# JuliaReinforcementLearning/ReinforcementLearning.jl

Hardware: NVIDIA H100
Metric: env-steps/sec at 65536 CartPole envs (full PPO iteration: rollout T=32 + GAE + 4 epochs x 4 minibatches) (higher is better)
Workload: dtype f32

## Files before the change

reinforcementlearning.jl_b200/csrc/nn_tc.cu:

```cuda
#include "nn.cuh"
#include "perm.cuh"
#include "tc_split.h"
#include "wgmma.cuh"

namespace {

constexpr int NT = 256;
constexpr int TM = 128;
constexpr int H = 64;
constexpr int G_F = 128;
constexpr int GW_S = 8 * G_F;
constexpr int WIMG_BYTES = 16 * GW_S;
constexpr float kScaleW = 64.0f;
constexpr float kLog2Pi = 1.8378770664093453f;

__device__ __forceinline__ float act_f(int act, float z) { return act == B200RL_ACT_RELU ? fmaxf(z, 0.f) : tanhf(z); }
__device__ __forceinline__ void split2(float a, float b, uint32_t& hi, uint32_t& lo) {
    const __half2 h = __floats2half2_rn(a, b);
    const float2 back = __half22float2(h);
    const __half2 l = __floats2half2_rn(a - back.x, b - back.y);
    hi = *reinterpret_cast<const uint32_t*>(&h);
    lo = *reinterpret_cast<const uint32_t*>(&l);
}
__device__ __forceinline__ float half_bits_to_float(uint32_t bits16) { return __half2float(__ushort_as_half((unsigned short)bits16)); }
__device__ __forceinline__ float softplus_f(float x) { return x > 0.f ? x + log1pf(expf(-x)) : log1pf(expf(x)); }
__device__ __forceinline__ float normlogpdf1(float mu, float sigma, float x) {
    float s = sigma + 1e-8f, v = s * s, dd = x - mu;
    return -0.5f * ((logf(v) + (dd * dd) / v) + kLog2Pi);
}
__device__ __forceinline__ uint32_t wimg_off(int n, int k) { return (uint32_t)((n >> 3) * GW_S + (k >> 3) * G_F + (n & 7) * 16 + (k & 7) * 2); }

constexpr int NT7 = 512;
constexpr int GF_T = 128;
constexpr int GS_T = 16 * GF_T;
constexpr int FIMG = 8 * GS_T;
constexpr float kScaleH = 64.0f, kScaleX = 64.0f;
constexpr int kNo = 2;

struct SmemBwd {
    static_assert(FIMG % 128 == 0 && WIMG_BYTES % 128 == 0 && (2 * GS_T) % 16 == 0, "operand images must stay 128-byte aligned");
    alignas(128) uint8_t FP_full[FIMG];
    alignas(128) uint8_t FP_lo[FIMG];
    alignas(128) uint8_t FH_lo[FIMG];
    alignas(128) uint8_t FH_full[FIMG];
    alignas(16) uint8_t FH_ones[2 * GS_T];
    alignas(128) uint8_t FQ_full[FIMG];
    alignas(128) uint8_t FQ_lo[FIMG];
    alignas(128) uint8_t B1[WIMG_BYTES];
    alignas(128) uint8_t XT[2][2 * GS_T];
    alignas(128) uint8_t AH_full[FIMG];
    alignas(128) uint8_t AH_lo[FIMG];
    alignas(16) float D[TM * H];
    float W1[kInMax * H];
    float b1[H], b2[H];
    float W3[H * kNo];
    float b3[kNo];
    float Zp[4 * kNo * TM];
    float Red[32];
    double RedD[16];
    float step_scale;
    alignas(8) uint64_t bar1;
    alignas(8) uint64_t bar2;
    alignas(8) uint64_t bar3;
    alignas(8) uint64_t bar4;
    float AccW2[64 * 65 + 64];
    float AccD4[64 * 9];
};
__device__ __forceinline__ int d_off(int s, int col) { return s * H + ((((col >> 2) ^ (s & 15))) << 2) + (col & 3); }
__device__ __forceinline__ void d_ld16(const float* D, int s, int f0, float (&v)[16]) {
#pragma unroll
    for (int u = 0; u < 4; ++u) {
        const float4 q4 = *reinterpret_cast<const float4*>(D + d_off(s, f0 + 4 * u));
        v[4 * u] = q4.x; v[4 * u + 1] = q4.y; v[4 * u + 2] = q4.z; v[4 * u + 3] = q4.w;
    }
}
template <int TB>
__device__ __forceinline__ void gemm_ts3(float (&d)[32], const uint8_t* a_hi, const uint8_t* a_lo, int h, uint64_t dB, uint32_t b_step) {
    const uint64_t dA = wg::make_desc(wg::smem_u32(a_hi) + 8 * h * GF_T, GS_T, GF_T), dAl = wg::make_desc(wg::smem_u32(a_lo) + 8 * h * GF_T, GS_T, GF_T);
    wg::fence();
#pragma unroll
    for (int k = 0; k < 4; ++k) {
        const uint32_t aa = k * 2 * GS_T, bb = k * b_step;
        wg::mma_m64n64k16<0, TB>(d, wg::desc_add(dA, aa), wg::desc_add(dB, bb), k ? 1u : 0u);
        wg::mma_m64n64k16<0, TB>(d, wg::desc_add(dA, aa), wg::desc_add(dB, 8 * GW_S + bb), 1u);
        wg::mma_m64n64k16<0, TB>(d, wg::desc_add(dAl, aa), wg::desc_add(dB, bb), 1u);
    }
    wg::commit();
    wg::wait_all();
}
__device__ __forceinline__ uint32_t fimg_off(int f, int s) { return (uint32_t)((f >> 3) * GS_T + (s >> 3) * GF_T + (s & 7) * 16 + (f & 7) * 2); }
__device__ __forceinline__ void store16_feat(uint8_t* img, int f0, int s, const uint32_t (&v)[8]) {
    uint8_t* p = img + fimg_off(f0, s);
    *reinterpret_cast<uint4*>(p) = make_uint4(v[0], v[1], v[2], v[3]);
    *reinterpret_cast<uint4*>(p + GS_T) = make_uint4(v[4], v[5], v[6], v[7]);
}
__device__ __forceinline__ float dact_f(int act, float h) { return act == B200RL_ACT_RELU ? (h > 0.f ? 1.f : 0.f) : 1.f - h * h; }

__device__ __forceinline__ uint32_t mix32(uint32_t h) {
    h ^= h >> 16; h *= 0x85EBCA6Bu; h ^= h >> 13; h *= 0xC2B2AE35u; h ^= h >> 16;
    return h;
}
using b200perm::perm_index;
using b200perm::perm_index_bits;
__device__ __forceinline__ float block_sum512(float v, float* red) {
#pragma unroll
    for (int o = 16; o > 0; o >>= 1) v += __shfl_xor_sync(0xffffffffu, v, o);
    __syncthreads();
    if ((threadIdx.x & 31) == 0) red[threadIdx.x >> 5] = v;
    __syncthreads();
    float t = 0.f;
    if (threadIdx.x == 0)
        for (int k = 0; k < NT7 / 32; ++k) t += red[k];
    return t;
}
__device__ __forceinline__ float sigmoid_f(float x) { return 1.f / (1.f + expf(-x)); }

__device__ __forceinline__ float lane_transpose_reduce32(float (&v)[32], int lane) {
#pragma unroll
    for (int st = 0; st < 5; ++st) {
        const int half = 16 >> st, off = 16 >> st;
        const bool upper = (lane & off) != 0;
#pragma unroll
        for (int n = 0; n < half; ++n) {
            float send = upper ? v[n] : v[n + half];
            float keep = upper ? v[n + half] : v[n];
            v[n] = keep + __shfl_xor_sync(0xffffffffu, send, off);
        }
    }
    return v[0];
}

__device__ __forceinline__ void worker_sync() { asm volatile("bar.sync 1, 512;" ::: "memory"); }
__device__ __forceinline__ void group_sync(int q) { asm volatile("bar.sync %0, 128;" ::"r"(5 + q) : "memory"); }
__device__ __forceinline__ void ready_arrive(int id) { asm volatile("bar.arrive %0, 640;" ::"r"(id) : "memory"); }
__device__ __forceinline__ void ready_wait(int id) { asm volatile("bar.sync %0, 640;" ::"r"(id) : "memory"); }
struct LossOut { float dz[kNo]; float l0, l1; };
__device__ __forceinline__ LossOut sample_loss(const MlpDesc& actor, int role, const AcHyper& hp, float inv_B, const float (&z)[kNo],
                                               float a_bits, float lp_old, float A, float ret) {
    LossOut r;
#pragma unroll
    for (int o = 0; o < kNo; ++o) r.dz[o] = 0.f;
    r.l0 = 0.f; r.l1 = 0.f;
    if (role == 1) {
        float err = ret - z[0];
        r.l0 = err * err;
        r.dz[0] = -2.0f * hp.w_critic * inv_B * err;
        return r;
    }
    float logp_a, gsel;
    if (!actor.heads2) {
        int na = actor.nout;
        float lp[kNo], pr[kNo];
        float m = -3.4e38f;
#pragma unroll
        for (int o = 0; o < kNo; ++o) if (o < na) m = fmaxf(m, z[o]);
        float se = 0.f;
#pragma unroll
        for (int o = 0; o < kNo; ++o) if (o < na) se += expf(z[o] - m);
        float ls = logf(se);
        float Hent = 0.f;
#pragma unroll
        for (int o = 0; o < kNo; ++o) {
            lp[o] = (z[o] - m) - ls;
            pr[o] = o < na ? expf(lp[o]) : 0.f;
            if (o < na) Hent -= pr[o] * lp[o];
        }
        int a = __float_as_int(a_bits) - 1;
        logp_a = 0.f;
#pragma unroll
        for (int o = 0; o < kNo; ++o) if (o == a) logp_a = lp[o];
        r.l1 = Hent;
        if (hp.algo == 0) {
            float ratio = expf(logp_a - lp_old);
            float u = ratio * A;
            float rc = fminf(fmaxf(ratio, 1.0f - hp.clip_range), 1.0f + hp.clip_range);
            float cc = rc * A;
            r.l0 = -fminf(u, cc);
            bool inside = ratio >= 1.0f - hp.clip_range && ratio <= 1.0f + hp.clip_range;
            gsel = (u < cc || inside) ? u : 0.f;
        } else {
            r.l0 = -(logp_a * A);
            gsel = A;
        }
        float dlogp = -hp.w_actor * inv_B * gsel;
#pragma unroll
        for (int o = 0; o < kNo; ++o)
            if (o < na) r.dz[o] = dlogp * ((o == a ? 1.f : 0.f) - pr[o]) + hp.w_entropy * inv_B * pr[o] * (lp[o] + Hent);
    } else {
        float mu = z[0], raw = z[1];
        float sp = softplus_f(raw);
        float sigma = fminf(fmaxf(sp, hp.min_sigma), hp.max_sigma);
        bool clamped = sp < hp.min_sigma || sp > hp.max_sigma;
        float a = a_bits;
        logp_a = normlogpdf1(mu, sigma, a);
        float Hent = logf(sigma) + 0.5f * (kLog2Pi + 1.0f);
        r.l1 = Hent;
        if (hp.algo == 0) {
            float ratio = expf(logp_a - lp_old);
            float u = ratio * A;
            float rc = fminf(fmaxf(ratio, 1.0f - hp.clip_range), 1.0f + hp.clip_range);
            float cc = rc * A;
            r.l0 = -fminf(u, cc);
            bool inside = ratio >= 1.0f - hp.clip_range && ratio <= 1.0f + hp.clip_range;
            gsel = (u < cc || inside) ? u : 0.f;
        } else {
            r.l0 = -(logp_a * A);
            gsel = A;
        }
        float dlogp = -hp.w_actor * inv_B * gsel;
        float sgm = sigma + 1e-8f, dd = a - mu;
        r.dz[0] = dlogp * (dd / (sgm * sgm));
        float dsig = dlogp * (-1.0f / sgm + (dd * dd) / (sgm * sgm * sgm)) - hp.w_entropy * inv_B * (1.0f / sigma);
        r.dz[1] = clamped ? 0.f : dsig * sigmoid_f(raw);
    }
    return r;
}

#ifdef B200RL_K7_TIMING
__device__ unsigned long long g_k7_phase[40];
__device__ int g_k7_watch = 0;
#define K7_T(i) do { if (tid == (g_k7_watch & 0xFFFF) && (int)blockIdx.x == (g_k7_watch >> 16)) { long long now_ = clock64(); g_k7_phase[i] += (unsigned long long)(now_ - tprev_); tprev_ = now_; } } while (0)
#else
#define K7_T(i) do { } while (0)
#endif
constexpr int NT7_ALL = NT7 + 128;
constexpr int kRegsMma = 64, kRegsWorker = 104;
static_assert(128 * kRegsMma + NT7 * kRegsWorker <= NT7_ALL * 96, "setmaxnreg split must fit the CTA's register allocation");
constexpr int kBarRdyA = 2, kBarRdyB = 3, kBarRdyC = 4;

template <int ACT>
__global__ void __launch_bounds__(NT7_ALL, 1)
ac_loss_grad_tc_kernel(MlpDesc actor, MlpDesc critic, const float* params , AcHyper hp, AcBatch b, float* partial,
                       float* __restrict__ loss_partial, int64_t np_total, float scale_base ,
                       AcStep st ,
                       int n_actor ) {
    extern __shared__ __align__(1024) unsigned char smem_raw[];
    SmemBwd& sm = *reinterpret_cast<SmemBwd*>(smem_raw);
    const int role = (int)blockIdx.x < n_actor ? 0 : 1;
    const int cta = role ? (int)blockIdx.x - n_actor : (int)blockIdx.x;
    const int nctas = role ? (int)gridDim.x - n_actor : n_actor;
    const int nrows = max(n_actor, (int)gridDim.x - n_actor);
    const float scale_p = scale_base * (role ? 4.0f : 64.0f);
    const MlpDesc d = role ? critic : actor;
    const int act = ACT >= 0 ? ACT : d.act;
    const bool relu = act == B200RL_ACT_RELU;
    const int64_t poff = role ? actor.nparams() : 0;
    const float* __restrict__ p = params + poff;
    const int tid = threadIdx.x, warp = tid >> 5, lane = tid & 31;
    const int q = warp & 3, c = (warp >> 2) & 3;
    const int s = 32 * q + lane;
    {
        const float* b1 = p + (int64_t)H * d.in;
        const float* W2 = b1 + H;
        const float* b2 = W2 + (int64_t)H * H;
        const float s1 = relu ? kScaleH : 1.0f;
        for (int k = tid; k < kInMax * H; k += NT7_ALL) sm.W1[k] = (k / H) < d.in ? p[k] * s1 : 0.f;
        for (int k = tid; k < H; k += NT7_ALL) { sm.b1[k] = b1[k] * s1; sm.b2[k] = b2[k]; }
        for (int k = tid; k < H * kNo; k += NT7_ALL) {
            int j = k / kNo, o = k % kNo;
            sm.W3[k] = o < d.nout ? p[head_w<false>(d, o, j)] : 0.f;
        }
        if (tid < kNo) sm.b3[tid] = tid < d.nout ? p[head_b<false>(d, tid)] : 0.f;
        for (int k = tid; k < H * H; k += NT7_ALL) {
            int o = k % H, i = k / H;
            const float w = W2[k] * kScaleW;
            const __half wh = __float2half_rn(w), wl = __float2half_rn(w - __half2float(wh));
            *reinterpret_cast<__half*>(sm.B1 + wimg_off(o, i)) = wh;
            *reinterpret_cast<__half*>(sm.B1 + wimg_off(H + o, i)) = wl;
        }
    }
    for (int k = tid; k < 2 * TM; k += NT7_ALL)
        *reinterpret_cast<uint4*>(sm.FH_ones + 16 * k) = make_uint4(k < TM ? 0x3C00u : 0u, 0u, 0u, 0u);
    if (tid == 32) {
        wg::mbar_init(&sm.bar1, 128); wg::mbar_init(&sm.bar2, 128); wg::mbar_init(&sm.bar3, 128); wg::mbar_init(&sm.bar4, 128);
    }
    wg::fence_proxy_async();
    __syncthreads();
    const float inv_s1 = 1.0f / (kScaleH * kScaleW), inv_s3 = 1.0f / (scale_p * kScaleH), inv_sp = 1.0f / scale_p, inv_s4 = 1.0f / (scale_p * kScaleX);
    const int64_t ntiles = (b.B + TM - 1) / TM;

    if (warp >= NT7 / 32) {
        asm volatile("setmaxnreg.dec.sync.aligned.u32 %0;" ::"n"(kRegsMma));
        const int t = tid - NT7, row0 = 16 * (t >> 5) + ((t & 31) >> 2), col0 = 2 * (t & 3);
        const uint64_t dB1k = wg::make_desc(wg::smem_u32(sm.B1), G_F, GW_S);
        const uint64_t dB1t = wg::make_desc(wg::smem_u32(sm.B1), GW_S, G_F);
        float dacc[32];
        auto store_d = [&](int h) {
#pragma unroll
            for (int j = 0; j < 8; ++j)
#pragma unroll
                for (int hh = 0; hh < 2; ++hh)
                    *reinterpret_cast<float2*>(sm.D + d_off(64 * h + row0 + 8 * hh, 8 * j + col0)) = make_float2(dacc[4 * j + 2 * hh], dacc[4 * j + 2 * hh + 1]);
        };
        auto gemm1 = [&](int h) { gemm_ts3<0>(dacc, sm.AH_full, sm.AH_lo, h, dB1k, 2 * G_F); };
        auto gemm2 = [&](int h) { gemm_ts3<1>(dacc, sm.FP_full, sm.FP_lo, h, dB1t, 2 * GW_S); };
        auto gemm3 = [&]() {
            const uint64_t dPh = wg::make_desc(wg::smem_u32(sm.FP_full), GF_T, GS_T), dPl = wg::make_desc(wg::smem_u32(sm.FP_lo), GF_T, GS_T);
            const uint64_t dHh = wg::make_desc(wg::smem_u32(sm.FH_full), GF_T, GS_T), dHl = wg::make_desc(wg::smem_u32(sm.FH_lo), GF_T, GS_T);
            wg::fence();
#pragma unroll
            for (int k = 0; k < 8; ++k) {
                const uint32_t a = k * 2 * GF_T;
                wg::mma_m64n64k16<1, 1>(dacc, wg::desc_add(dPh, a), wg::desc_add(dHh, a), k ? 1u : 0u);
                wg::mma_m64n64k16<1, 1>(dacc, wg::desc_add(dPl, a), wg::desc_add(dHh, a), 1u);
                wg::mma_m64n64k16<1, 1>(dacc, wg::desc_add(dPh, a), wg::desc_add(dHl, a), 1u);
            }
            wg::commit();
            wg::wait_all();
#pragma unroll
            for (int j = 0; j < 8; ++j)
#pragma unroll
                for (int hh = 0; hh < 2; ++hh)
#pragma unroll
                    for (int e = 0; e < 2; ++e) sm.AccW2[(row0 + 8 * hh) * 65 + 8 * j + col0 + e] += dacc[4 * j + 2 * hh + e];
            const uint64_t dOnes = wg::make_desc(wg::smem_u32(sm.FH_ones), GF_T, GS_T);
            float d8[4] = {0.f, 0.f, 0.f, 0.f};
            wg::fence();
#pragma unroll
            for (int k = 0; k < 8; ++k) {
                const uint32_t a = k * 2 * GF_T;
                wg::mma_m64n8k16<1, 1>(d8, wg::desc_add(dPh, a), wg::desc_add(dOnes, a), k ? 1u : 0u);
                wg::mma_m64n8k16<1, 1>(d8, wg::desc_add(dPl, a), wg::desc_add(dOnes, a), 1u);
            }
            wg::commit();
            wg::wait_all();
            if (col0 == 0) {
                sm.AccW2[64 * 65 + row0] += d8[0];
                sm.AccW2[64 * 65 + row0 + 8] += d8[2];
            }
        };
        auto gemm4 = [&](int buf) {
            const uint64_t dQh = wg::make_desc(wg::smem_u32(sm.FQ_full), GF_T, GS_T), dQl = wg::make_desc(wg::smem_u32(sm.FQ_lo), GF_T, GS_T);
            const uint64_t dX = wg::make_desc(wg::smem_u32(sm.XT[buf]), GF_T, GS_T);
            float d4[4] = {0.f, 0.f, 0.f, 0.f};
            wg::fence();
#pragma unroll
            for (int k = 0; k < 8; ++k) {
                const uint32_t a = k * 2 * GF_T;
                wg::mma_m64n8k16<1, 1>(d4, wg::desc_add(dQh, a), wg::desc_add(dX, a), k ? 1u : 0u);
                wg::mma_m64n8k16<1, 1>(d4, wg::desc_add(dQh, a), wg::desc_add(dX, GS_T + a), 1u);
                wg::mma_m64n8k16<1, 1>(d4, wg::desc_add(dQl, a), wg::desc_add(dX, a), 1u);
            }
            wg::commit();
            wg::wait_all();
#pragma unroll
            for (int hh = 0; hh < 2; ++hh)
#pragma unroll
                for (int e = 0; e < 2; ++e)
                    if (col0 + e < 5) sm.AccD4[(row0 + 8 * hh) * 9 + col0 + e] += d4[2 * hh + e];
        };
        if (cta < ntiles) {
            ready_wait(kBarRdyB);
            for (int h = 0; h < 2; ++h) { gemm1(h); store_d(h); }
            wg::mbar_arrive(&sm.bar1);
        }
        int buf = 0;
        for (int64_t tile = cta; tile < ntiles; tile += nctas, buf ^= 1) {
            const bool has_next = tile + nctas < ntiles;
            ready_wait(kBarRdyA);
            for (int h = 0; h < 2; ++h) { gemm2(h); store_d(h); }
            wg::mbar_arrive(&sm.bar2);
            gemm3();
            wg::mbar_arrive(&sm.bar3);
            if (has_next) {
                ready_wait(kBarRdyB);
                gemm1(0);
            }
            ready_wait(kBarRdyC);
            if (has_next) {
                store_d(0);
                gemm1(1);
                store_d(1);
                wg::mbar_arrive(&sm.bar1);
            }
            gemm4(buf);
            wg::mbar_arrive(&sm.bar4);
        }
    } else {
    asm volatile("setmaxnreg.inc.sync.aligned.u32 %0;" ::"n"(kRegsWorker));
    float g3[2][16];
    float gb3a0 = 0.f, gb3a1 = 0.f;
#pragma unroll
    for (int k = 0; k < 16; ++k) { g3[0][k] = 0.f; g3[1][k] = 0.f; }
    float l0 = 0.f, l1 = 0.f;
    float mean = 0.f, inv_std = 1.f;
    if (hp.normalize_adv && b.norm2) { mean = b.norm2[0]; inv_std = b.norm2[1]; }
    uint32_t ph1 = 0, ph2 = 0, ph3 = 0, ph4 = 0;
    bool gemm4_pending = false;
    int xbuf = 0;
#ifdef B200RL_K7_TIMING
    long long tprev_ = clock64();
#endif
    const int pbits = b200perm::perm_bits(b.perm_n);
    const uint32_t pkey = ac_perm_key(b);
    auto index_of = [&](int64_t t) -> int32_t {
        const int64_t j = t * TM + s;
        if (t >= ntiles || j >= b.B) return -1;
        return b.idx ? b.idx[j] : (int32_t)perm_index_bits((uint32_t)(b.perm_offset + j), b.perm_n, pkey, pbits);
    };
    auto request = [&](int32_t g, float (&x)[kInMax], float (&a)[4]) {
#pragma unroll
        for (int k = 0; k < kInMax; ++k) { x[k] = 0.f; a[k] = 0.f; }
        if (g < 0) return;
        if (b.rec) {
            const float4 v0 = b.rec[2 * (int64_t)g], v1 = b.rec[2 * (int64_t)g + 1];
            x[0] = v0.x; x[1] = v0.y; x[2] = v0.z; x[3] = v0.w;
            a[0] = v1.x; a[1] = v1.y; a[2] = v1.z; a[3] = v1.w;
        } else {
#pragma unroll
            for (int i = 0; i < kInMax; ++i)
                if (i < b.ns) x[i] = b.states[(int64_t)b.ns * g + i];
            a[0] = reinterpret_cast<const float*>(b.actions)[g];
            a[1] = b.logp_old ? b.logp_old[g] : 0.f;
            a[2] = b.adv[g];
            a[3] = b.ret[g];
        }
    };
    float pfx[kInMax] = {0.f, 0.f, 0.f, 0.f}, pfa[4] = {0.f, 0.f, 0.f, 0.f};
    float aux[4] = {0.f, 0.f, 0.f, 0.f};
    int32_t gi_next = -1;
    bool gemm3_pending = false;
    float* const out = partial + (int64_t)cta * np_total + poff;
    float* const gW1 = out;
    float* const gb1 = out + (int64_t)H * d.in;
    float* const gW2 = gb1 + H;
    float* const gb2 = gW2 + (int64_t)H * H;
    for (int k = tid; k < 64 * 65 + 64; k += NT7) sm.AccW2[k] = 0.f;
    for (int k = tid; k < 64 * 9; k += NT7) sm.AccD4[k] = 0.f;
    float xo[kInMax];
    auto publish = [&](int64_t t) {
#pragma unroll
        for (int i = 0; i < kInMax; ++i) xo[i] = pfx[i];
        aux[0] = pfa[0];
        aux[1] = role == 0 ? pfa[1] : 0.f;
        aux[2] = role == 0 ? (hp.normalize_adv ? (pfa[2] - mean) * inv_std : pfa[2]) : 0.f;
        aux[3] = role == 0 ? 0.f : pfa[3];
        if (c == 0) {
            uint32_t h01, l01, h23, l23;
            split2(xo[0] * kScaleX, xo[1] * kScaleX, h01, l01);
            split2(xo[2] * kScaleX, xo[3] * kScaleX, h23, l23);
            uint8_t* xt = sm.XT[xbuf] + fimg_off(0, s);
            *reinterpret_cast<uint4*>(xt) = make_uint4(h01, h23, 0x3C00u, 0u);
            *reinterpret_cast<uint4*>(xt + GS_T) = make_uint4(l01, l23, 0u, 0u);
        }
        K7_T(16);
        xbuf ^= 1;
        request(gi_next, pfx, pfa);
        gi_next = index_of(t + 2 * nctas);
        K7_T(17);
    };
    uint32_t h1pos = 0, h1pos_tile = 0;
    auto layer1 = [&]() {
        uint32_t pos = 0;
        uint32_t hi8[8], lo8[8];
#pragma unroll
        for (int ch = 0; ch < 4; ++ch) {
            const int f0 = 16 * c + 4 * ch;
            float4 bb = *reinterpret_cast<const float4*>(sm.b1 + f0);
            float h[4] = {bb.x, bb.y, bb.z, bb.w};
#pragma unroll
            for (int k = 0; k < kInMax; ++k) {
                float4 w = *reinterpret_cast<const float4*>(sm.W1 + k * H + f0);
                h[0] = fmaf(w.x, xo[k], h[0]); h[1] = fmaf(w.y, xo[k], h[1]); h[2] = fmaf(w.z, xo[k], h[2]); h[3] = fmaf(w.w, xo[k], h[3]);
            }
            if (relu) {
#pragma unroll
                for (int e = 0; e < 4; ++e) { pos |= (h[e] > 0.f ? 1u : 0u) << (4 * ch + e); h[e] = fmaxf(h[e], 0.f); }
            } else {
#pragma unroll
                for (int e = 0; e < 4; ++e) h[e] = act_f(act, h[e]) * kScaleH;
            }
            split2(h[0], h[1], hi8[2 * ch], lo8[2 * ch]);
            split2(h[2], h[3], hi8[2 * ch + 1], lo8[2 * ch + 1]);
        }
        h1pos = pos;
        store16_feat(sm.AH_full, 16 * c, s, hi8);
        store16_feat(sm.AH_lo, 16 * c, s, lo8);
    };
    if (cta < ntiles) {
        request(index_of(cta), pfx, pfa);
        gi_next = index_of(cta + nctas);
        publish(cta);
        layer1();
        wg::fence_proxy_async();
        ready_arrive(kBarRdyB);
    }
#ifdef B200RL_K7_TIMING
    tprev_ = clock64();
#endif
    for (int64_t tile = cta; tile < ntiles; tile += nctas) {
        const bool has_next = tile + nctas < ntiles;
        wg::mbar_wait(&sm.bar1, ph1);
        ph1 ^= 1u;
        K7_T(0);
        float h2[16];
        {
            float v[16];
            d_ld16(sm.D, s, 16 * c, v);
            float zp[kNo] = {0.f, 0.f};
#pragma unroll
            for (int k = 0; k < 16; ++k) {
                const int f = 16 * c + k;
                h2[k] = act_f(act, fmaf(v[k], inv_s1, sm.b2[f]));
                float2 w = *reinterpret_cast<const float2*>(sm.W3 + f * kNo);
                zp[0] = fmaf(w.x, h2[k], zp[0]); zp[1] = fmaf(w.y, h2[k], zp[1]);
            }
#pragma unroll
            for (int o = 0; o < kNo; ++o) sm.Zp[(c * kNo + o) * TM + s] = zp[o];
        }
        K7_T(1);
        group_sync(q);
        K7_T(2);
        {
            float z[kNo];
#pragma unroll
            for (int o = 0; o < kNo; ++o)
                z[o] = sm.b3[o] + ((sm.Zp[o * TM + s] + sm.Zp[(kNo + o) * TM + s]) + (sm.Zp[(2 * kNo + o) * TM + s] + sm.Zp[(3 * kNo + o) * TM + s]));
            const bool valid = (tile * TM + s) < b.B;
            LossOut lo_ = sample_loss(actor, role, hp, b.inv_B, z, aux[0], aux[1], aux[2], aux[3]);
            float dz[kNo];
#pragma unroll
            for (int o = 0; o < kNo; ++o) dz[o] = valid ? lo_.dz[o] : 0.f;
            if (c == 0 && valid) { l0 += lo_.l0; l1 += lo_.l1; gb3a0 += dz[0]; gb3a1 += dz[1]; }
            const float dzs0 = dz[0] * scale_p, dzs1 = dz[1] * scale_p;
            float dp[16];
#pragma unroll
            for (int k = 0; k < 16; ++k) {
                const int f = 16 * c + k;
                float2 w = *reinterpret_cast<const float2*>(sm.W3 + f * kNo);
                const float dh = fmaf(w.x, dzs0, w.y * dzs1);
                dp[k] = relu ? (h2[k] > 0.f ? dh : 0.f) : dh * (1.f - h2[k] * h2[k]);
                g3[0][k] = fmaf(dz[0], h2[k], g3[0][k]);
                g3[1][k] = fmaf(dz[1], h2[k], g3[1][k]);
            }
            uint32_t hi8[8], lo8[8];
#pragma unroll
            for (int m = 0; m < 8; ++m) split2(dp[2 * m], dp[2 * m + 1], hi8[m], lo8[m]);
            K7_T(3);
            if (gemm3_pending) {
                wg::mbar_wait(&sm.bar3, ph3);
                ph3 ^= 1u;
                gemm3_pending = false;
            }
            K7_T(4);
            store16_feat(sm.FP_full, 16 * c, s, hi8);
            store16_feat(sm.FP_lo, 16 * c, s, lo8);
            {
                const uint32_t off = fimg_off(16 * c, s);
                const uint4 h0 = *reinterpret_cast<const uint4*>(sm.AH_full + off), h1 = *reinterpret_cast<const uint4*>(sm.AH_full + off + GS_T);
                const uint4 l0 = *reinterpret_cast<const uint4*>(sm.AH_lo + off), l1 = *reinterpret_cast<const uint4*>(sm.AH_lo + off + GS_T);
                *reinterpret_cast<uint4*>(sm.FH_full + off) = h0; *reinterpret_cast<uint4*>(sm.FH_full + off + GS_T) = h1;
                *reinterpret_cast<uint4*>(sm.FH_lo + off) = l0; *reinterpret_cast<uint4*>(sm.FH_lo + off + GS_T) = l1;
            }
        }
        K7_T(5);
        wg::fence_proxy_async();
        ready_arrive(kBarRdyA);
        gemm3_pending = true;
        K7_T(6);
        K7_T(7);
        h1pos_tile = h1pos;
        if (has_next) {
            if (gemm4_pending) {
                wg::mbar_wait(&sm.bar4, ph4);
                ph4 ^= 1u;
                gemm4_pending = false;
            }
            publish(tile + nctas);
            K7_T(8);
            K7_T(9);
            layer1();
            wg::fence_proxy_async();
            K7_T(10);
            ready_arrive(kBarRdyB);
            K7_T(11);
        }
        K7_T(12);
        wg::mbar_wait(&sm.bar2, ph2);
        ph2 ^= 1u;
        K7_T(13);
        {
            float v[16];
            d_ld16(sm.D, s, 16 * c, v);
#pragma unroll
            for (int k = 0; k < 16; ++k) v[k] *= 1.0f / kScaleW;
            if (relu) {
#pragma unroll
                for (int k = 0; k < 16; ++k) v[k] = ((h1pos_tile >> k) & 1u) ? v[k] : 0.f;
            } else {
                const float inv_h = 1.0f / kScaleH;
#pragma unroll
                for (int g8 = 0; g8 < 2; ++g8) {
                    const uint32_t off = fimg_off(16 * c + 8 * g8, s);
                    const uint4 hv = *reinterpret_cast<const uint4*>(sm.FH_full + off), lv = *reinterpret_cast<const uint4*>(sm.FH_lo + off);
                    const uint32_t hw[4] = {hv.x, hv.y, hv.z, hv.w}, lw[4] = {lv.x, lv.y, lv.z, lv.w};
#pragma unroll
                    for (int m = 0; m < 4; ++m) {
                        const float2 hf = __half22float2(*reinterpret_cast<const __half2*>(&hw[m])), lf = __half22float2(*reinterpret_cast<const __half2*>(&lw[m]));
                        v[8 * g8 + 2 * m] *= dact_f(act, (hf.x + lf.x) * inv_h);
                        v[8 * g8 + 2 * m + 1] *= dact_f(act, (hf.y + lf.y) * inv_h);
                    }
                }
            }
            if (gemm4_pending) {
                wg::mbar_wait(&sm.bar4, ph4);
                ph4 ^= 1u;
                gemm4_pending = false;
            }
            {
                uint32_t hi8[8], lo8[8];
#pragma unroll
                for (int m = 0; m < 8; ++m) split2(v[2 * m], v[2 * m + 1], hi8[m], lo8[m]);
                store16_feat(sm.FQ_full, 16 * c, s, hi8);
                store16_feat(sm.FQ_lo, 16 * c, s, lo8);
            }
            gemm4_pending = true;
        }
        K7_T(14);
#ifdef B200RL_K7_TIMING
        if (tid == (g_k7_watch & 0xFFFF) && (int)blockIdx.x == (g_k7_watch >> 16)) g_k7_phase[15] += 1;
#endif
        wg::fence_proxy_async();
        ready_arrive(kBarRdyC);
    }
    if (gemm3_pending) wg::mbar_wait(&sm.bar3, ph3);
    if (gemm4_pending) wg::mbar_wait(&sm.bar4, ph4);
    worker_sync();
    for (int k = tid; k < H * H; k += NT7) gW2[k] = sm.AccW2[(k & 63) * 65 + (k >> 6)] * inv_s3;
    if (tid < H) {
        gb2[tid] = sm.AccW2[64 * 65 + tid] * inv_sp;
        gb1[tid] = sm.AccD4[tid * 9 + 4] * inv_sp;
        for (int i = 0; i < d.in; ++i) gW1[tid + H * i] = sm.AccD4[tid * 9 + i] * inv_s4;
    }
    if (cta >= (int)gridDim.x - nctas) {
        const int64_t ooff = role ? 0 : actor.nparams(), on = role ? actor.nparams() : critic.nparams();
        float* orow = partial + (int64_t)cta * np_total + ooff;
        for (int64_t kk = tid; kk < on; kk += NT7) orow[kk] = 0.f;
    }
    float* red = reinterpret_cast<float*>(sm.FP_full);
    static_assert(offsetof(SmemBwd, XT) - offsetof(SmemBwd, FP_full) >= (2 * TM * 65 + 2 * 8 * 64) * 4, "drain scratch");
    {
        constexpr int RS = 65;
        float* seg = red + 2 * TM * RS;
#pragma unroll
        for (int k = 0; k < 16; ++k) {
            red[0 * TM * RS + s * RS + 16 * c + k] = g3[0][k];
            red[1 * TM * RS + s * RS + 16 * c + k] = g3[1][k];
        }
        worker_sync();
        {
            const int col = tid & 63, g = tid >> 6;
#pragma unroll
            for (int m = 0; m < 2; ++m) {
                float a = 0.f;
#pragma unroll
                for (int ss = 0; ss < 16; ++ss) a += red[m * TM * RS + (16 * g + ss) * RS + col];
                seg[(m * 8 + g) * 64 + col] = a;
            }
        }
        worker_sync();
        if (tid < 2 * H) {
            const int m = tid >> 6, col = tid & 63;
            float a = 0.f;
#pragma unroll
            for (int g = 0; g < 8; ++g) a += seg[(m * 8 + g) * 64 + col];
            if (m < d.nout) out[head_w<false>(d, m, col)] = a;
        }
        worker_sync();
    }
    if (c == 0) { red[s] = gb3a0; red[TM + s] = gb3a1; }
    worker_sync();
    if (warp < d.nout) {
        float a = (red[warp * TM + lane] + red[warp * TM + 32 + lane]) + (red[warp * TM + 64 + lane] + red[warp * TM + 96 + lane]);
#pragma unroll
        for (int o = 16; o > 0; o >>= 1) a += __shfl_xor_sync(0xffffffffu, a, o);
        if (lane == 0) out[head_b<false>(d, warp)] = a;
    }
    float t0 = l0, t1 = l1;
#pragma unroll
    for (int o = 16; o > 0; o >>= 1) { t0 += __shfl_xor_sync(0xffffffffu, t0, o); t1 += __shfl_xor_sync(0xffffffffu, t1, o); }
    worker_sync();
    if (lane == 0) { sm.Red[warp] = t0; sm.Red[16 + warp] = t1; }
    worker_sync();
    if (tid == 0) {
        float a0 = 0.f, a1 = 0.f;
        for (int k = 0; k < 16; ++k) { a0 += sm.Red[k]; a1 += sm.Red[16 + k]; }
        float* lp = loss_partial + (int64_t)blockIdx.x * 4;
        lp[0] = role ? 0.f : a0; lp[1] = role ? 0.f : a1; lp[2] = role ? a0 : 0.f; lp[3] = 0.f;
    }
    if (st.params) {
        const unsigned int G = gridDim.x;
        K7_T(24);
        worker_sync();
        K7_T(25);
        if (tid == 0) {
            __threadfence();
            atomicAdd(st.counter, 1u);
            unsigned int spins = 0;
            while (*reinterpret_cast<volatile unsigned int*>(st.counter) < G)
                if (++spins > (1u << 26)) __trap();
            __threadfence();
        }
        worker_sync();
        K7_T(26);
        const int per = (int)((np_total + G - 1) / G);
        const int64_t k = (int64_t)blockIdx.x * per + tid;
        const bool mine = tid < per && k < np_total;
        const unsigned int seq = st.tab.nranks > 1 ? *st.seq_ptr + 1u : 0u;
        float* stage = reinterpret_cast<float*>(sm.FP_full);
        const int nstage = per * nrows;
        const int64_t k0 = (int64_t)blockIdx.x * per;
        {
            constexpr int kMaxStage = 10;
            float t[kMaxStage];
#pragma unroll
            for (int j = 0; j < kMaxStage; ++j) {
                const int e = tid + j * NT7;
                const int row = e / per, col = e - row * per;
                t[j] = (e < nstage && k0 + col < np_total) ? __ldcg(partial + (int64_t)row * np_total + k0 + col) : 0.f;
            }
#pragma unroll
            for (int j = 0; j < kMaxStage; ++j) {
                const int e = tid + j * NT7;
                if (e < nstage) stage[e] = t[j];
            }
        }
        float* lstage = stage + nstage;
        if (blockIdx.x == 0) {
            float t[2];
#pragma unroll
            for (int j = 0; j < 2; ++j) t[j] = tid + j * NT7 < 4 * (int)G ? __ldcg(loss_partial + tid + j * NT7) : 0.f;
#pragma unroll
            for (int j = 0; j < 2; ++j) if (tid + j * NT7 < 4 * (int)G) lstage[tid + j * NT7] = t[j];
        }
        float m_k = 0.f, v_k = 0.f, p_k = 0.f;
        if (mine) { m_k = st.m[k]; v_k = st.v[k]; p_k = st.params[k]; }
        worker_sync();
        K7_T(27);
        float gk = 0.f;
        if (mine) {
            for (int c0 = 0; c0 < nrows; c0 += 8) {
                float t[8];
#pragma unroll
                for (int j = 0; j < 8; ++j) t[j] = c0 + j < nrows ? stage[(c0 + j) * per + tid] : 0.f;
#pragma unroll
                for (int j = 0; j < 8; ++j) if (c0 + j < nrows) gk += t[j];
            }
        }
        float lsum = 0.f;
        const bool loss_thread = blockIdx.x == 0 && tid < 4;
        if (loss_thread) {
            for (unsigned int c0 = 0; c0 < G; c0 += 8) {
                float t[8];
#pragma unroll
                for (int j = 0; j < 8; ++j) t[j] = c0 + j < G ? lstage[(c0 + j) * 4 + tid] : 0.f;
#pragma unroll
                for (int j = 0; j < 8; ++j) if (c0 + j < G) lsum += t[j];
            }
        }
        if (st.tab.nranks > 1) {
            const unsigned slot = seq & 1u;
            if (mine) p2p_push(st.tab, 0, slot, (size_t)k, __float_as_uint(gk), seq);
            if (loss_thread) p2p_push(st.tab, 0, slot, (size_t)np_total + tid, __float_as_uint(lsum), seq);
            float acc = 0.f, lacc = 0.f;
            for (int r = 0; r < st.tab.nranks; ++r) {
                if (mine) acc += r == st.tab.rank ? gk : __uint_as_float(p2p_recv(st.tab, 0, slot, r, (size_t)k, seq));
                if (loss_thread) lacc += r == st.tab.rank ? lsum : __uint_as_float(p2p_recv(st.tab, 0, slot, r, (size_t)np_total + tid, seq));
            }
            gk = acc; lsum = lacc;
        }
        if (loss_thread) {
            if (st.loss_out4) st.loss_out4[tid] = lsum;
            if (st.stats_row) st.stats_row[tid] = lsum;
        }
        double sq = (double)gk * (double)gk;
#pragma unroll
        for (int o = 16; o > 0; o >>= 1) sq += __shfl_xor_sync(0xffffffffu, sq, o);
        if (lane == 0) sm.RedD[warp] = sq;
        worker_sync();
        K7_T(28);
        if (warp == 0) {
            if (lane == 0) {
                double t = 0.0;
                for (int w = 0; w < NT7 / 32; ++w) t += sm.RedD[w];
                st.cta_sumsq[blockIdx.x] = t;
                __threadfence();
                atomicAdd(st.counter + 1, 1u);
                unsigned int spins = 0;
                while (*reinterpret_cast<volatile unsigned int*>(st.counter + 1) < G)
                    if (++spins > (1u << 26)) __trap();
                __threadfence();
            }
            __syncwarp();
            K7_T(29);
            double part[8];
#pragma unroll
            for (int j = 0; j < 8; ++j) part[j] = (unsigned)(lane + 32 * j) < G ? __ldcg(st.cta_sumsq + lane + 32 * j) : 0.0;
            double tot = 0.0;
#pragma unroll
            for (int j = 0; j < 8; ++j) tot += part[j];
#pragma unroll
            for (int o = 16; o > 0; o >>= 1) tot += __shfl_xor_sync(0xffffffffu, tot, o);
            if (lane == 0) {
                const float gn = (float)sqrt(tot);
                float sc = 1.0f;
                if (st.max_norm > 0.f && st.max_norm <= gn) sc = st.max_norm / fmaxf(st.max_norm, gn);
                sm.step_scale = sc;
                if (blockIdx.x == 0) {
                    if (st.gnorm_out) *st.gnorm_out = gn;
                    if (st.stats_row) st.stats_row[4] = gn;
                }
            }
        }
        worker_sync();
        K7_T(30);
        const float bt1 = st.beta_t[0], bt2 = st.beta_t[1];
        if (mine) {
            gk *= sm.step_scale;
            st.grad[k] = gk;
            const float mk = st.b1 * m_k + (1.0f - st.b1) * gk;
            const float vk = st.b2 * v_k + (1.0f - st.b2) * (gk * gk);
            st.m[k] = mk; st.v[k] = vk;
            st.params[k] = p_k - mk / (1.0f - bt1) / (sqrtf(vk / (1.0f - bt2)) + st.eps) * st.lr;
        }
        worker_sync();
        if (tid == 0) {
            if (atomicAdd(st.counter + 2, 1u) + 1u == G) {
                st.beta_t[0] = bt1 * st.b1; st.beta_t[1] = bt2 * st.b2;
                st.counter[0] = 0u; st.counter[1] = 0u; st.counter[2] = 0u;
                if (st.tab.nranks > 1) *st.seq_ptr = seq;
                if (st.tick) *st.tick += 1u;
            }
        }
        K7_T(31);
    }
    }
    __syncthreads();
}

}

int nn_tc_actor_ctas(int grid, const MlpDesc& actor, const AcHyper& hp, int64_t ntiles) {
    static int forced = -2;
    if (forced == -2) { const char* e = getenv("B200RL_K7_ACTOR_CTAS"); forced = e ? atoi(e) : -1; }
    if (forced > 0 && forced < grid) return forced;
    (void)hp;
    return b200rl_tc_actor_ctas(grid, actor.heads2 != 0, ntiles);
}
int nn_tc_partial_rows(int grid, const MlpDesc& actor, const AcHyper& hp, int64_t B) {
    const int na = nn_tc_actor_ctas(grid, actor, hp, (B + TM - 1) / TM);
    return na > grid - na ? na : grid - na;
}
bool nn_tc_bwd_supported(const MlpDesc& actor, const MlpDesc& critic) {
    return actor.H == 64 && critic.H == 64 && actor.in <= kInMax && actor.nout <= 2 && critic.nout == 1;
}
int nn_tc_ac_loss_grad(b200rl_ctx* ctx, int grid, const MlpDesc& actor, const MlpDesc& critic, const float* params, const AcHyper& hp,
                       const AcBatch& b, float* partial, float* loss_partial, int64_t np, const AcStep* step) {
    AcStep st = {};
    const int n_actor = nn_tc_actor_ctas(grid, actor, hp, (b.B + TM - 1) / TM);
    if (step) {
        st = *step;
        const int64_t per = (np + grid - 1) / grid;
        const int rows = n_actor > grid - n_actor ? n_actor : grid - n_actor;
        REQUIRE(st.params == params && per <= NT7 && grid <= ctx->sm_count && per * rows <= 10 * NT7 && 4 * grid <= 2 * NT7 && grid <= 256, B200RL_ERR_UNSUPPORTED,
                "fused optimiser step: bad configuration");
    }
    size_t smem = sizeof(SmemBwd) + 128;
    static unsigned long long attr_devices = 0;
    if (first_use_on_device(attr_devices, ctx->device)) {
        CUDA_TRY(cudaFuncSetAttribute(ac_loss_grad_tc_kernel<B200RL_ACT_RELU>, cudaFuncAttributeMaxDynamicSharedMemorySize, (int)smem));
        CUDA_TRY(cudaFuncSetAttribute(ac_loss_grad_tc_kernel<B200RL_ACT_TANH>, cudaFuncAttributeMaxDynamicSharedMemorySize, (int)smem));
        CUDA_TRY(cudaFuncSetAttribute(ac_loss_grad_tc_kernel<-1>, cudaFuncAttributeMaxDynamicSharedMemorySize, (int)smem));
    }
    const float scale_base = exp2f(floorf(log2f(1.0f / b.inv_B)));
    if (actor.act == critic.act && actor.act == B200RL_ACT_RELU)
        ac_loss_grad_tc_kernel<B200RL_ACT_RELU><<<grid, NT7_ALL, smem, ctx->stream>>>(actor, critic, params, hp, b, partial, loss_partial, np, scale_base, st, n_actor);
    else if (actor.act == critic.act && actor.act == B200RL_ACT_TANH)
        ac_loss_grad_tc_kernel<B200RL_ACT_TANH><<<grid, NT7_ALL, smem, ctx->stream>>>(actor, critic, params, hp, b, partial, loss_partial, np, scale_base, st, n_actor);
    else
        ac_loss_grad_tc_kernel<-1><<<grid, NT7_ALL, smem, ctx->stream>>>(actor, critic, params, hp, b, partial, loss_partial, np, scale_base, st, n_actor);
    LAUNCH_CHECK(ctx);
    return B200RL_OK;
}

#ifdef B200RL_K7_TIMING
extern "C" int b200rl_debug_k7_watch(int tid) {
    cudaDeviceSynchronize();
    return cudaMemcpyToSymbol(g_k7_watch, &tid, sizeof tid) == cudaSuccess ? 0 : -1;
}
extern "C" int b200rl_debug_k7_phases(unsigned long long* out16, int reset) {
    cudaDeviceSynchronize();
    if (cudaMemcpyFromSymbol(out16, g_k7_phase, sizeof(unsigned long long) * 40) != cudaSuccess) return -1;
    if (reset) { unsigned long long z[24] = {0}; cudaMemcpyToSymbol(g_k7_phase, z, sizeof z); }
    return 0;
}
#endif
```

Baseline: 279.0 million.

## Prefetch both GEMM1 halves early into a separate D1n buffer in K7

```diff
diff --git a/reinforcementlearning.jl_b200/csrc/nn_tc.cu b/reinforcementlearning.jl_b200/csrc/nn_tc.cu
--- a/reinforcementlearning.jl_b200/csrc/nn_tc.cu
+++ b/reinforcementlearning.jl_b200/csrc/nn_tc.cu
@@ -43,7 +43,7 @@
     alignas(128) uint8_t FP_lo[FIMG];
     alignas(128) uint8_t FH_lo[FIMG];
     alignas(128) uint8_t FH_full[FIMG];
-    alignas(16) uint8_t FH_ones[2 * GS_T];
+    alignas(16) uint8_t FH_ones[GS_T];
     alignas(128) uint8_t FQ_full[FIMG];
     alignas(128) uint8_t FQ_lo[FIMG];
     alignas(128) uint8_t B1[WIMG_BYTES];
@@ -51,13 +51,15 @@
     alignas(128) uint8_t AH_full[FIMG];
     alignas(128) uint8_t AH_lo[FIMG];
     alignas(16) float D[TM * H];
+    alignas(16) float D1n[(TM / 2) * H];
     float W1[kInMax * H];
     float b1[H], b2[H];
     float W3[H * kNo];
     float b3[kNo];
-    float Zp[4 * kNo * TM];
-    float Red[32];
-    double RedD[16];
+    union {
+        float Zp[4 * kNo * TM];
+        struct { float Red[32]; double RedD[16]; } fin;
+    };
     float step_scale;
     alignas(8) uint64_t bar1;
     alignas(8) uint64_t bar2;
@@ -66,6 +68,7 @@
     float AccW2[64 * 65 + 64];
     float AccD4[64 * 9];
 };
+static_assert(sizeof(SmemBwd) + 128 <= 227 * 1024, "K7's shared memory (+ 128 B for aligning the base) must fit the 227 KB a CTA can opt in to on H100");
 __device__ __forceinline__ int d_off(int s, int col) { return s * H + ((((col >> 2) ^ (s & 15))) << 2) + (col & 3); }
 __device__ __forceinline__ void d_ld16(const float* D, int s, int f0, float (&v)[16]) {
 #pragma unroll
@@ -217,11 +220,14 @@
 }
 
 #ifdef B200RL_K7_TIMING
-__device__ unsigned long long g_k7_phase[40];
+constexpr int kK7Phases = 48, kK7MaxCtas = 256;
+__device__ unsigned long long g_k7_phase[kK7Phases + kK7MaxCtas];
 __device__ int g_k7_watch = 0;
 #define K7_T(i) do { if (tid == (g_k7_watch & 0xFFFF) && (int)blockIdx.x == (g_k7_watch >> 16)) { long long now_ = clock64(); g_k7_phase[i] += (unsigned long long)(now_ - tprev_); tprev_ = now_; } } while (0)
+#define K7_M(i) do { if (tid == NT7 && (int)blockIdx.x == (g_k7_watch >> 16)) { long long now_ = clock64(); g_k7_phase[32 + (i)] += (unsigned long long)(now_ - tprev_); tprev_ = now_; } } while (0)
 #else
 #define K7_T(i) do { } while (0)
+#define K7_M(i) do { } while (0)
 #endif
 constexpr int NT7_ALL = NT7 + 128;
 constexpr int kRegsMma = 64, kRegsWorker = 104;
@@ -249,6 +255,9 @@
     const int tid = threadIdx.x, warp = tid >> 5, lane = tid & 31;
     const int q = warp & 3, c = (warp >> 2) & 3;
     const int s = 32 * q + lane;
+#ifdef B200RL_K7_TIMING
+    const long long t_start = clock64();
+#endif
     {
         const float* b1 = p + (int64_t)H * d.in;
         const float* W2 = b1 + H;
@@ -269,8 +278,7 @@
             *reinterpret_cast<__half*>(sm.B1 + wimg_off(H + o, i)) = wl;
         }
     }
-    for (int k = tid; k < 2 * TM; k += NT7_ALL)
-        *reinterpret_cast<uint4*>(sm.FH_ones + 16 * k) = make_uint4(k < TM ? 0x3C00u : 0u, 0u, 0u, 0u);
+    for (int k = tid; k < TM; k += NT7_ALL) *reinterpret_cast<uint4*>(sm.FH_ones + 16 * k) = make_uint4(0x3C00u, 0u, 0u, 0u);
     if (tid == 32) {
         wg::mbar_init(&sm.bar1, 128); wg::mbar_init(&sm.bar2, 128); wg::mbar_init(&sm.bar3, 128); wg::mbar_init(&sm.bar4, 128);
     }
@@ -285,12 +293,12 @@
         const uint64_t dB1k = wg::make_desc(wg::smem_u32(sm.B1), G_F, GW_S);
         const uint64_t dB1t = wg::make_desc(wg::smem_u32(sm.B1), GW_S, G_F);
         float dacc[32];
-        auto store_d = [&](int h) {
+        auto store_d = [&](float* dst, int h) {
 #pragma unroll
             for (int j = 0; j < 8; ++j)
 #pragma unroll
                 for (int hh = 0; hh < 2; ++hh)
-                    *reinterpret_cast<float2*>(sm.D + d_off(64 * h + row0 + 8 * hh, 8 * j + col0)) = make_float2(dacc[4 * j + 2 * hh], dacc[4 * j + 2 * hh + 1]);
+                    *reinterpret_cast<float2*>(dst + d_off(64 * h + row0 + 8 * hh, 8 * j + col0)) = make_float2(dacc[4 * j + 2 * hh], dacc[4 * j + 2 * hh + 1]);
         };
         auto gemm1 = [&](int h) { gemm_ts3<0>(dacc, sm.AH_full, sm.AH_lo, h, dB1k, 2 * G_F); };
         auto gemm2 = [&](int h) { gemm_ts3<1>(dacc, sm.FP_full, sm.FP_lo, h, dB1t, 2 * GW_S); };
@@ -351,30 +359,42 @@
         };
         if (cta < ntiles) {
             ready_wait(kBarRdyB);
-            for (int h = 0; h < 2; ++h) { gemm1(h); store_d(h); }
+            gemm1(1); store_d(sm.D1n, 0);
+            gemm1(0); store_d(sm.D, 0);
             wg::mbar_arrive(&sm.bar1);
         }
         int buf = 0;
+#ifdef B200RL_K7_TIMING
+        long long tprev_ = clock64();
+#endif
         for (int64_t tile = cta; tile < ntiles; tile += nctas, buf ^= 1) {
             const bool has_next = tile + nctas < ntiles;
             ready_wait(kBarRdyA);
-            for (int h = 0; h < 2; ++h) { gemm2(h); store_d(h); }
+            K7_M(0);
+            for (int h = 0; h < 2; ++h) { gemm2(h); store_d(sm.D, h); }
             wg::mbar_arrive(&sm.bar2);
+            K7_M(1);
             gemm3();
             wg::mbar_arrive(&sm.bar3);
+            K7_M(2);
             if (has_next) {
                 ready_wait(kBarRdyB);
+                K7_M(3);
+                gemm1(1);
+                store_d(sm.D1n, 0);
                 gemm1(0);
+                K7_M(4);
             }
             ready_wait(kBarRdyC);
+            K7_M(5);
             if (has_next) {
-                store_d(0);
-                gemm1(1);
-                store_d(1);
+                store_d(sm.D, 0);
                 wg::mbar_arrive(&sm.bar1);
             }
+            K7_M(6);
             gemm4(buf);
             wg::mbar_arrive(&sm.bar4);
+            K7_M(7);
         }
     } else {
     asm volatile("setmaxnreg.inc.sync.aligned.u32 %0;" ::"n"(kRegsWorker));
@@ -496,7 +516,7 @@
         float h2[16];
         {
             float v[16];
-            d_ld16(sm.D, s, 16 * c, v);
+            d_ld16(s < 64 ? sm.D : sm.D1n, s & 63, 16 * c, v);
             float zp[kNo] = {0.f, 0.f};
 #pragma unroll
             for (int k = 0; k < 16; ++k) {
@@ -625,6 +645,9 @@
     }
     if (gemm3_pending) wg::mbar_wait(&sm.bar3, ph3);
     if (gemm4_pending) wg::mbar_wait(&sm.bar4, ph4);
+#ifdef B200RL_K7_TIMING
+    if (tid == 0 && blockIdx.x < kK7MaxCtas) g_k7_phase[kK7Phases + blockIdx.x] += (unsigned long long)(clock64() - t_start);
+#endif
     worker_sync();
     for (int k = tid; k < H * H; k += NT7) gW2[k] = sm.AccW2[(k & 63) * 65 + (k >> 6)] * inv_s3;
     if (tid < H) {
@@ -680,11 +703,11 @@
 #pragma unroll
     for (int o = 16; o > 0; o >>= 1) { t0 += __shfl_xor_sync(0xffffffffu, t0, o); t1 += __shfl_xor_sync(0xffffffffu, t1, o); }
     worker_sync();
-    if (lane == 0) { sm.Red[warp] = t0; sm.Red[16 + warp] = t1; }
+    if (lane == 0) { sm.fin.Red[warp] = t0; sm.fin.Red[16 + warp] = t1; }
     worker_sync();
     if (tid == 0) {
         float a0 = 0.f, a1 = 0.f;
-        for (int k = 0; k < 16; ++k) { a0 += sm.Red[k]; a1 += sm.Red[16 + k]; }
+        for (int k = 0; k < 16; ++k) { a0 += sm.fin.Red[k]; a1 += sm.fin.Red[16 + k]; }
         float* lp = loss_partial + (int64_t)blockIdx.x * 4;
         lp[0] = role ? 0.f : a0; lp[1] = role ? 0.f : a1; lp[2] = role ? a0 : 0.f; lp[3] = 0.f;
     }
@@ -776,13 +799,13 @@
         double sq = (double)gk * (double)gk;
 #pragma unroll
         for (int o = 16; o > 0; o >>= 1) sq += __shfl_xor_sync(0xffffffffu, sq, o);
-        if (lane == 0) sm.RedD[warp] = sq;
+        if (lane == 0) sm.fin.RedD[warp] = sq;
         worker_sync();
         K7_T(28);
         if (warp == 0) {
             if (lane == 0) {
                 double t = 0.0;
-                for (int w = 0; w < NT7 / 32; ++w) t += sm.RedD[w];
+                for (int w = 0; w < NT7 / 32; ++w) t += sm.fin.RedD[w];
                 st.cta_sumsq[blockIdx.x] = t;
                 __threadfence();
                 atomicAdd(st.counter + 1, 1u);
@@ -888,10 +911,10 @@
     cudaDeviceSynchronize();
     return cudaMemcpyToSymbol(g_k7_watch, &tid, sizeof tid) == cudaSuccess ? 0 : -1;
 }
-extern "C" int b200rl_debug_k7_phases(unsigned long long* out16, int reset) {
+extern "C" int b200rl_debug_k7_phases(unsigned long long* out, int reset) {
     cudaDeviceSynchronize();
-    if (cudaMemcpyFromSymbol(out16, g_k7_phase, sizeof(unsigned long long) * 40) != cudaSuccess) return -1;
-    if (reset) { unsigned long long z[24] = {0}; cudaMemcpyToSymbol(g_k7_phase, z, sizeof z); }
+    if (cudaMemcpyFromSymbol(out, g_k7_phase, sizeof g_k7_phase) != cudaSuccess) return -1;
+    if (reset) { static const unsigned long long z[kK7Phases + kK7MaxCtas] = {}; cudaMemcpyToSymbol(g_k7_phase, z, sizeof z); }
     return 0;
 }
 #endif
```

Result: faster. 289.0 million, median of 6 (+3.6%).
